# dvnam1605/MAACO-path-planing

Hardware: AMD Instinct MI355X
Metric: agent-fitness-evals/sec on 512x512 grid (higher is better)
Workload: dtype f64

## Files before the change

include/pathfit.h:

```cpp
#ifndef PATHFIT_H
#define PATHFIT_H
#include <stdint.h>
#ifdef __cplusplus
extern "C" {
#endif

#define PF_ST_OK 0
#define PF_ST_INFEASIBLE 1
#define PF_ST_STEP_CAP 2
#define PF_ST_OVERFLOW 3
#define PF_ST_KEPT 4

#define PF_ASTAR_REF 0
#define PF_ASTAR_MPA 1
#define PF_ASTAR_DIJKSTRA 2

typedef struct pf_handle pf_handle;

typedef struct {
  int32_t variant;
  int32_t restrict_policy;
  double w_turn, w_safe, min_safe, diag_pen;
} pf_score_params;

// ... 102 lines not shown
int pf_mpa_setup(pf_handle* h, const pf_mpa_params* p, const pf_score_params* sp);
int pf_mpa_phase_batch(pf_handle* h, int32_t phase, double CF, int32_t iter, uint64_t seed, int32_t n,
                       int32_t path_cap, const int32_t* d_pop_cells, const int32_t* d_pop_len,
                       const double* d_pop_stats, const int32_t* d_gidx, const int32_t* d_slot,
                       const int32_t* d_elite_cells, int32_t elite_len, const double* d_elite_stats,
                       int32_t* d_out_cells, int32_t* d_out_len, double* d_out_stats, int32_t* d_status);
int pf_mpa_fads_batch(pf_handle* h, double CF, int32_t iter, uint64_t seed, int32_t n, int32_t path_cap,
                      const int32_t* d_gidx, const int32_t* d_slot, int32_t* d_pop_cells, int32_t* d_pop_len,
                      double* d_pop_stats, int32_t* d_status);
int pf_mpa_iter_batch(pf_handle* h, int32_t phase, double CF, int32_t iter, uint64_t seed, int32_t n, int32_t path_cap,
                      int32_t* d_pop_cells, int32_t* d_pop_len, double* d_pop_stats, const int32_t* d_gidx,
                      const int32_t* d_slot, const int32_t* d_elite_cells, int32_t elite_len, const double* d_elite_stats,
                      int32_t* d_c1_cells, int32_t* d_c1_len, double* d_c1_stats, int32_t* d_c2_cells, int32_t* d_c2_len,
                      double* d_c2_stats, int32_t* d_status);
int pf_mpa_iter_ahead(pf_handle* h, int32_t depth, const int32_t* phases, const double* CFs, const int32_t* iters, uint64_t seed, int32_t n,
                      int32_t path_cap, int32_t* d_pop_cells, int32_t* d_pop_len, double* d_pop_stats, const int32_t* d_gidx,
                      const int32_t* d_slot, const int32_t* d_elite_cells, int32_t elite_len, const double* d_elite_stats,
                      int32_t* d_c1_cells, int32_t* d_c1_len, double* d_c1_stats, int32_t* d_c2_cells, int32_t* d_c2_len,
                      double* d_c2_stats, int32_t* d_status, int32_t* accepted);
int pf_mpa_ahead_take(pf_handle* h, int32_t iter, const int32_t* d_slot, int32_t* d_pop_cells, int32_t* d_pop_len, double* d_pop_stats,
                      int32_t* accepted);
int pf_mpa_ahead_level_bufs(pf_handle* h, void** out7);
int pf_mpa_ahead_drop(pf_handle* h);
int pf_mpa_ahead_stats(pf_handle* h, int64_t* out6);
int pf_mpa_rebuild_batch(pf_handle* h, int32_t iter, uint64_t seed, int32_t n, int32_t path_cap,
                         const int32_t* d_pop_cells, const int32_t* d_pop_len, const double* d_pop_stats,
                         const int32_t* d_elite_cells, int32_t elite_len, const int32_t* d_idx,
                         const int32_t* d_is_levy, const double* d_scale, const int32_t* d_agent,
                         int32_t* d_out_cells, int32_t* d_out_len, double* d_out_stats, int32_t* d_status);
int pf_mpa_memory(pf_handle* h, int32_t n, int32_t path_cap, const int32_t* d_slot, const int32_t* d_cand_cells,
                  const int32_t* d_cand_len, const double* d_cand_stats, int32_t* d_pop_cells, int32_t* d_pop_len,
                  double* d_pop_stats);

typedef struct pf_mpa_batch pf_mpa_batch;
int pf_mpa_batch_create(pf_handle* h, const pf_mpa_params* p, const pf_score_params* sp, int32_t K, const int32_t* starts,
                        const int32_t* targets, const uint64_t* seeds, pf_mpa_batch** out);
void pf_mpa_batch_destroy(pf_mpa_batch* b);
int pf_mpa_batch_init_path(pf_mpa_batch* b, int32_t k, int32_t* cells_out, int32_t cap, int32_t* len_out, double* stats5);
int pf_mpa_batch_create_ms(pf_mpa_batch* b, double* out3);
int pf_mpa_batch_sort(pf_mpa_batch* b, const double* d_pop_stats, int32_t* d_order);
int pf_mpa_batch_pick_elite(pf_mpa_batch* b, int32_t path_cap, const int32_t* d_pop_cells, const int32_t* d_pop_len,
                            const double* d_pop_stats, const int32_t* d_order);
int pf_mpa_batch_iterate(pf_mpa_batch* b, int32_t phase, double CF, int32_t iter, int32_t path_cap, int32_t* d_pop_cells,
                         int32_t* d_pop_len, double* d_pop_stats, const int32_t* d_order, int32_t* d_c1_cells, int32_t* d_c1_len,
                         double* d_c1_stats, int32_t* d_c2_cells, int32_t* d_c2_len, double* d_c2_stats, int32_t* d_status);
int pf_mpa_batch_best_rows(pf_mpa_batch* b, const double* d_pop_stats, const int32_t* d_order, double* out);
int pf_mpa_batch_read_path(pf_mpa_batch* b, int32_t k, int32_t slot, int32_t path_cap, const int32_t* d_pop_cells,
// ... 87 lines not shown
```

maaco-path-planing_amd/csrc/pathfit.hip:

```cpp
#include <hip/hip_runtime.h>
#include <dlfcn.h>
#include <rccl/rccl.h>
#include <math.h>
#include <stdio.h>
#include <stdlib.h>
#include <string.h>
#include <algorithm>
#include <chrono>
#include <queue>
#include <string>
#include <vector>

#include "../../include/pathfit.h"
#include "pf_astar.h"
#include "pf_device.h"
#include "pf_score.h"

using namespace pf;

#define DOM_MAACO 1
#define DOM_MPA 2
#define DOM_PSO 3
#define DOM_MPA_FADS 5
#define DOM_GA 4
// ... 1005 lines not shown
  Open O = make_open(smem, p.c.S, p.c.tier2);
  Slot s = slot_load(p.c, p.c.G.R * p.c.G.C);
  AStat tot = {0, 0, 0, 0, 0, 0};
  unsigned long long cells = 0, ovf = 0;
  for (;;) {
    const int a = next_agent(p.c, p.n, lane);
    if (a < 0) break;
    mpa_fads_item(p, a, s, O, tot, cells, ovf, lane);
  }
  slot_store(p.c, s, lane);
  flush_counters(p.c.cnt, tot, cells, ovf, lane);
}

struct MpaSweepArgs { MpaPhaseArgs ph; MpaFadsArgs fd; };
struct __attribute__((aligned(16))) MpaJob {
  const int* src;
  int n0;
  int astart, g0, g1;
  int kind;
  int aux;
};
struct MpaRes { int n, rc; };

PF_DEV void mpa_plan_item(const MpaPhaseArgs& p, const MpaFadsArgs& f, bool isph, int a, int item, MpaJob* jobs, MpaRes* res) {
  const Grid& G = p.c.G;
  const int lane = lane_id();
  MpaJob j; j.src = nullptr; j.n0 = 0; j.astart = 0; j.g0 = -1; j.g1 = p.m.target; j.kind = 0; j.aux = isph ? 4 : 0;
  unsigned long long pruned_n = 0;
  if (isph) {
    const MpaPlan pl = mpa_plan(p, a);
    const int2 pr = p.prop[a];
    const int idx = first_i(pr.x);
    if (idx >= 0) {
      const int* mod = pl.mod;
      const int cur = mod[idx];
      const int inter = first_i(pr.y);
      bool pruned = false;
      if (p.m.dt) {
        double pre = 0.0;
        for (int i = lane; i < idx; i += 64) {
          const int dd = mod[i + 1] - mod[i];
          pre += (dd == 1 || dd == -1 || dd == G.C || dd == -G.C) ? 1.0 : PF_SQRT2;
        }
        pre = wave_sum_d(pre);
        double lb = p.m.dt[cur];
        if (G.occ[inter] != 1 && inter != cur) {
          const int r0 = row_of(G, cur), r1 = row_of(G, inter);
          const long dr_ = r1 - r0, dc_ = (inter - r1 * G.C) - (cur - r0 * G.C);
          lb = fmin(lb, __builtin_sqrt((double)(dr_ * dr_ + dc_ * dc_)) + p.m.dt[inter]);
        }
        lb = (pre + lb) * (1.0 - 1e-9);
        const double prey_fit = pl.prey_stats[4];
        pruned = lb >= prey_fit && (mod == pl.prey || pl.mod_stats[4] >= prey_fit);
      }
      if (pruned) pruned_n = 1;
      else if (idx + 1 > p.path_cap) j.aux = 3;
      else {
        j.kind = 1; j.src = mod; j.n0 = idx + 1; j.astart = cur;
        j.g0 = (G.occ[inter] != 1 && inter != cur) ? inter : -1;
      }
    }
  } else {
    Rng g; g.init(f.seed, DOM_MPA_FADS, (unsigned long long)f.iter, (unsigned long long)f.gidx[a]);
    if (g.random() < f.m.fads) {
      if (g.random() < f.CF) {
        const int rr_ = (int)g.randint(0, G.R - 1);
        const int rc_ = (int)g.randint(0, G.C - 1);
        const int node = rr_ * G.C + rc_;
        bool pruned = false;
        if (f.m.dt && G.occ[node] != 1) {
          pruned = (f.m.ds[node] + f.m.dt[node]) * (1.0 - 1e-9) >= f.pop_stats[(size_t)f.slot[a] * 5 + 4];
          if (pruned) pruned_n = 1;
        }
        if (G.occ[node] != 1 && !pruned) { j.kind = 2; j.n0 = 0; j.astart = f.m.start; j.g0 = node; }
      } else if (f.init_len > 0) j.aux = f.init_len > f.path_cap ? 3 : 1;
    }
  }
  if (lane == 0) {
    jobs[item] = j;
    MpaRes r; r.n = 0; r.rc = 1; res[item] = r;
    if (pruned_n) atomicAdd(&p.c.cnt->pruned, pruned_n);
  }
}
__global__ __launch_bounds__(64) void k_mpa_plan(MpaSweepArgs q, MpaJob* jobs, MpaRes* res) {
  const MpaPhaseArgs& p = q.ph;
  const int item = blockIdx.x;
  if (item >= 2 * p.n) return;
  const bool isph = item < p.n;
  mpa_plan_item(p, q.fd, isph, isph ? item : item - p.n, item, jobs, res);
}

struct MpaSearchArgs { Common c; const MpaJob* jobs; MpaRes* res; int n_items, path_cap; int* ph_cells; int* fd_cells; int n; };

template <bool PR>
__global__ __launch_bounds__(PR ? 128 : 64) __attribute__((amdgpu_waves_per_eu(3, 8))) void k_mpa_search(MpaSearchArgs p) {
  extern __shared__ __attribute__((aligned(16))) char smem[];
  const int lane = lane_id();
  const Grid& G = p.c.G;
  const int RC = G.R * G.C;
#ifdef PF_TWO_WAVE
  if (PR) {
    const int wave = (int)(threadIdx.x >> 6);
    if (wave == 0) pr_init_ctl(smem, lane);
    __syncthreads();
// ... 2740 lines not shown
  CK(hipMemsetAsync(h->d_scan3, 0, sizeof(int), h->stream));
  hipLaunchKernelGGL(k_plan_decode_multi<>, dim3((a.n + 255) / 256), dim3(256), 0, h->stream, a.c.G, a.n, a.W, a.wp_cells, a.wp_pos, d_start, d_target,
                     est, (int*)h->d_scan3);
  CK(hipGetLastError());
  return 0;
}
static int decode_multi_bad_ends(pf_handle* h, int* bad) {
  if (d2h_one(h, (const int*)h->d_scan3, bad)) return -1;
  h->d2h_small += 1;
  return 0;
}
static int decode_multi_launch(pf_handle* h, const DecodeArgs& a, const int* d_start, const int* d_target, int n) {
  DecodeMultiArgs m;
  m.c = a.c; m.sp = a.sp; m.do_score = a.do_score; m.n = a.n; m.W = a.W; m.path_cap = a.path_cap; m.start = d_start; m.target = d_target;
  m.wp_cells = a.wp_cells; m.wp_pos = a.wp_pos; m.cells = a.cells; m.len = a.len; m.status = a.status; m.stats = a.stats;
  return plateau_map(h) ? launch_with_retry(h, k_decode_multi<true>, m, n) : launch_with_retry(h, k_decode_multi<false>, m, n);
}

#include "pf_mpa_ahead.h"

struct MpaAhead {
  int *c1_cells = nullptr, *c1_len = nullptr, *c2_cells = nullptr, *c2_len = nullptr, *status = nullptr;
  double *c1_stats = nullptr, *c2_stats = nullptr;
  size_t rows_cap = 0; int row_cells = 0;
  unsigned long long* d_ctl = nullptr;
  int planned = 0, valid = 0, next = 0;
  int prev_accepted = 0;
  int iters[PF_AHEAD_MAX] = {};
  int n = 0, path_cap = 0;
  const int* slot = nullptr; int* pop_cells = nullptr; int* pop_len = nullptr; double* pop_stats = nullptr;
  int last_level = -1;
  long long sweeps = 0, levels = 0, served = 0, stale = 0;
};
static void mpa_ahead_drop(pf_handle* h) {
  MpaAhead* S = h->ahead;
  if (!S) return;
  S->planned = S->valid = S->next = 0; S->last_level = -1;
}
static void mpa_ahead_free(pf_handle* h) {
  MpaAhead* S = h->ahead;
  if (!S) return;
  void* ptrs[] = {S->c1_cells, S->c1_len, S->c1_stats, S->c2_cells, S->c2_len, S->c2_stats, S->status, S->d_ctl};
  for (void* q : ptrs) if (q) (void)hipFree(q);
  delete S;
  h->ahead = nullptr;
}
static int mpa_ahead_state(pf_handle* h) {
  if (!h->ahead) h->ahead = new MpaAhead();
  if (!h->ahead->d_ctl) CK(hipMalloc(&h->ahead->d_ctl, sizeof(unsigned long long) * (1 + PF_AHEAD_MAX)));
  return 0;
}
static int mpa_ahead_rows(pf_handle* h, size_t rows, int path_cap) {
  MpaAhead* S = h->ahead;
  if (rows <= S->rows_cap && path_cap == S->row_cells) return 0;
  CK(hipStreamSynchronize(h->stream));
  void** slots[] = {(void**)&S->c1_cells, (void**)&S->c1_len, (void**)&S->c1_stats, (void**)&S->c2_cells, (void**)&S->c2_len,
                    (void**)&S->c2_stats, (void**)&S->status};
  for (void** q : slots) if (*q) { (void)hipFree(*q); *q = nullptr; }
  S->rows_cap = 0;
  CK(hipMalloc(&S->c1_cells, sizeof(int) * rows * path_cap)); CK(hipMalloc(&S->c2_cells, sizeof(int) * rows * path_cap));
  CK(hipMalloc(&S->c1_len, sizeof(int) * rows)); CK(hipMalloc(&S->c2_len, sizeof(int) * rows)); CK(hipMalloc(&S->status, sizeof(int) * rows));
  CK(hipMalloc(&S->c1_stats, sizeof(double) * 5 * rows)); CK(hipMalloc(&S->c2_stats, sizeof(double) * 5 * rows));
  S->rows_cap = rows; S->row_cells = path_cap;
  return 0;
}

extern "C" {

int pf_mpa_iter_ahead(pf_handle* h, int32_t depth, const int32_t* phases, const double* CFs, const int32_t* iters, uint64_t seed, int32_t n,
                      int32_t path_cap, int32_t* d_pop_cells, int32_t* d_pop_len, double* d_pop_stats, const int32_t* d_gidx,
                      const int32_t* d_slot, const int32_t* d_elite_cells, int32_t elite_len, const double* d_elite_stats,
                      int32_t* d_c1_cells, int32_t* d_c1_len, double* d_c1_stats, int32_t* d_c2_cells, int32_t* d_c2_len,
                      double* d_c2_stats, int32_t* d_status, int32_t* accepted) {
  if (!h) return -2;
  if (!h->mpa_ready) return failmsg(h, "pf_mpa_iter_ahead: call pf_mpa_setup first");
  if (depth < 1 || depth > PF_AHEAD_MAX || !phases || !CFs || !iters || n <= 0 || (int64_t)depth * n > (1 << 28) || path_cap < 2 || !d_pop_cells ||
      !d_pop_len || !d_pop_stats || !d_gidx || !d_slot || !d_elite_cells || !d_elite_stats || !d_c1_cells || !d_c1_len || !d_c1_stats ||
      !d_c2_cells || !d_c2_len || !d_c2_stats || !d_status || !accepted)
    return failmsg(h, "pf_mpa_iter_ahead: bad arguments");
  for (int d = 0; d < depth; ++d) if (phases[d] < 1 || phases[d] > 3) return failmsg(h, "pf_mpa_iter_ahead: bad arguments");
  MpaBase base;
  if (mpa_solo_base(h, &base) || mpa_ahead_state(h)) return -1;
  mpa_ahead_drop(h);
  MpaAhead* S = h->ahead;
  const int D = depth, DN = D * n;
  if (D > 1) {
    if (mpa_ahead_rows(h, (size_t)DN, path_cap)) return -1;
    d_c1_cells = S->c1_cells; d_c1_len = S->c1_len; d_c1_stats = S->c1_stats;
    d_c2_cells = S->c2_cells; d_c2_len = S->c2_len; d_c2_stats = S->c2_stats; d_status = S->status;
  }
  MpaLevels ls; ls.D = D; ls.N = n;
  for (int d = 0; d < PF_AHEAD_MAX; ++d) { const int e = d < D ? d : 0; ls.lv[d].phase = phases[e]; ls.lv[d].iter = iters[e]; ls.lv[d].CF = CFs[e]; }
  MpaSweepArgs a;
  a.ph = mpa_phase_args(base, phases[0], CFs[0], iters[0], seed, n, path_cap, d_pop_cells, d_pop_len, d_pop_stats, d_gidx, d_slot, d_c1_cells,
                        d_c1_len, d_c1_stats, d_status);
  a.ph.elite_cells = d_elite_cells; a.ph.elite_len = elite_len; a.ph.elite_stats = d_elite_stats;
  if (elite_len < 0) { if (ensure_elite_buf(h)) return -1; a.ph.elite_len_dev = h->d_elite_len; }
  a.fd = mpa_fads_args(base, CFs[0], iters[0], seed, n, path_cap, d_pop_cells, d_pop_len, d_pop_stats, d_gidx, d_slot, d_status);
  a.fd.init_cells = h->d_init_cells; a.fd.init_len = h->init_len; a.fd.init_stats = h->d_init_stats;
  a.fd.cand_cells = d_c2_cells; a.fd.cand_len = d_c2_len; a.fd.cand_stats = d_c2_stats;
  int prc = 0;
  if (make_queue(h, 2 * DN, [&](float* est) {
        if (D == 1) {
          prc = mpa_launch_propose(h, a.ph, est);
          hipLaunchKernelGGL(k_plan_mpa_fads, dim3((n + 255) / 256), dim3(256), 0, h->stream, a.fd, est + n);
          return;
        }
        prc = mpa_prop_scratch(h, a.ph, DN);
        if (prc) return;
        hipLaunchKernelGGL(k_mpa_estimates_ahead<>, dim3((2 * DN + 255) / 256), dim3(256), 0, h->stream, a.ph, a.fd, ls, est);
      })) return -1;
  if (prc) return -1;
  {
    std::vector<int> list;
    if (mpa_doubt_list(h, a.ph, list)) return -1;
    for (int g : list) {
      const int d = g / n;
      MpaPhaseArgs v = a.ph;
      level_view(v, ls, d);
      if (mpa_resolve_one(h, v, g - d * n)) return -1;
    }
  }
#ifdef PF_TWO_WAVE
  const bool pr = g_two_wave != 0 && !plateau_map(h);
#else
  const bool pr = false;
#endif
  unsigned long long* const ctl = S->d_ctl;
  if (D > 1) CK(hipMemsetAsync(ctl, 0, sizeof(unsigned long long) * (1 + PF_AHEAD_MAX), h->stream));
  DevCounters dc;
  if (mpa_launch_sweep(h, a, DN, pr,
      [&](MpaJob* jobs, MpaRes* jres) {
        if (D == 1) hipLaunchKernelGGL(k_mpa_plan, dim3(2 * n), dim3(64), 0, h->stream, a, jobs, jres);
        else hipLaunchKernelGGL(k_mpa_plan_ahead<>, dim3(2 * DN), dim3(64), 0, h->stream, a, ls, jobs, jres);
      },
      [&](const MpaJob* jobs, const MpaRes* jres) {
        if (D == 1) hipLaunchKernelGGL(k_mpa_finish, dim3(2 * n), dim3(64), 0, h->stream, a, jobs, jres);
        else hipLaunchKernelGGL(k_mpa_finish_ahead<>, dim3(2 * DN), dim3(64), 0, h->stream, a, ls, jobs, jres, ctl + 1);
      },
      [&] { hipLaunchKernelGGL(k_mpa_apply_count<>, dim3(n), dim3(64), 0, h->stream, n, path_cap, d_slot, (const int*)d_c1_cells, (const int*)d_c1_len,
                               (const double*)d_c1_stats, (const int*)d_c2_cells, (const int*)d_c2_len, (const double*)d_c2_stats, d_pop_cells,
                               d_pop_len, d_pop_stats, &h->d_cnt->done); },
      &dc)) return -1;
  *accepted = (int32_t)dc.done;
  if (D == 1) return 0;
  unsigned long long hc[1 + PF_AHEAD_MAX];
  if (d2h_bytes(h, ctl, hc, sizeof(unsigned long long) * (size_t)(1 + D))) return -1;
  h->d2h_small += 1;
  h->last.overflow_agents = (long long)hc[1];
  S->sweeps += 1; S->levels += D - 1;
  S->planned = D; S->valid = D; S->next = 1; S->prev_accepted = (int)dc.done; S->last_level = 0;
  for (int d = D - 1; d >= 1; --d) if (hc[1 + d] > 0) S->valid = d;
  if (hc[1] > 0) S->valid = 1;
  for (int d = 0; d < D; ++d) S->iters[d] = iters[d];
  S->n = n; S->path_cap = path_cap; S->slot = d_slot; S->pop_cells = d_pop_cells; S->pop_len = d_pop_len; S->pop_stats = d_pop_stats;
  return 0;
}

int pf_mpa_ahead_take(pf_handle* h, int32_t iter, const int32_t* d_slot, int32_t* d_pop_cells, int32_t* d_pop_len, double* d_pop_stats,
                      int32_t* accepted) {
  if (!h) return -2;
  if (!accepted) return failmsg(h, "pf_mpa_ahead_take: bad arguments");
  *accepted = -1;
  MpaAhead* S = h->ahead;
  if (!S || S->next >= S->planned) return 0;
  const int d = S->next;
  if (d >= S->valid || S->prev_accepted != 0 || S->iters[d] != iter || d_slot != S->slot || d_pop_cells != S->pop_cells ||
      d_pop_len != S->pop_len || d_pop_stats != S->pop_stats) {
    S->stale += 1;
    mpa_ahead_drop(h);
    return 0;
  }
  CK(hipSetDevice(h->device));
  const size_t o = (size_t)d * (size_t)S->n;
  const int n = S->n, cap = S->path_cap;
  CK(hipMemsetAsync(S->d_ctl, 0, sizeof(unsigned long long), h->stream));
  hipLaunchKernelGGL(k_mpa_apply_count<>, dim3(n), dim3(64), 0, h->stream, n, cap, d_slot, (const int*)(S->c1_cells + o * cap),
                     (const int*)(S->c1_len + o), (const double*)(S->c1_stats + o * 5), (const int*)(S->c2_cells + o * cap), (const int*)(S->c2_len + o),
                     (const double*)(S->c2_stats + o * 5), d_pop_cells, d_pop_len, d_pop_stats, S->d_ctl);
  CK(hipGetLastError());
  unsigned long long acc64 = 0;
  if (d2h_one(h, S->d_ctl, &acc64)) return -1;
  h->d2h_small += 1;
  const int acc = (int)acc64;
  S->prev_accepted = acc; S->next = d + 1; S->last_level = d; S->served += 1;
  h->last = pf_counters{}; h->last_ms = 0.f;
  *accepted = acc;
  return 0;
}

int pf_mpa_ahead_level_bufs(pf_handle* h, void** out7) {
  if (!h) return -2;
  if (!out7) return failmsg(h, "pf_mpa_ahead_level_bufs: bad arguments");
  for (int i = 0; i < 7; ++i) out7[i] = nullptr;
  const MpaAhead* S = h->ahead;
  if (!S || S->last_level < 0) return 0;
  const size_t o = (size_t)S->last_level * (size_t)S->n;
  out7[0] = S->c1_cells + o * S->path_cap; out7[1] = S->c1_len + o; out7[2] = S->c1_stats + o * 5;
  out7[3] = S->c2_cells + o * S->path_cap; out7[4] = S->c2_len + o; out7[5] = S->c2_stats + o * 5; out7[6] = S->status + o;
  return 0;
}

int pf_mpa_ahead_drop(pf_handle* h) { if (!h) return -2; mpa_ahead_drop(h); return 0; }

int pf_mpa_ahead_stats(pf_handle* h, int64_t* out6) {
  if (!h) return -2;
  if (!out6) return failmsg(h, "pf_mpa_ahead_stats: bad arguments");
  const MpaAhead* S = h->ahead;
  out6[0] = g_mpa_lookahead; out6[1] = g_mpa_lookahead_always;
  out6[2] = S ? S->sweeps : 0; out6[3] = S ? S->levels : 0; out6[4] = S ? S->served : 0; out6[5] = S ? S->stale : 0;
  return 0;
}

}

#include "pf_pso_batch.h"
extern "C" {

int pf_pso_update_batch(pf_handle* h, int32_t n, int32_t K, int32_t N, int32_t W, double w, double c1, double c2, double max_vel, uint64_t iter,
                        const uint64_t* d_seeds, const int32_t* d_tab, const int32_t* d_starts, const int32_t* d_targets, const double* d_pos,
                        const double* d_vel, const double* d_pbest, const double* d_gbest, double* d_s_pos, double* d_s_vel, int32_t* d_s_start,
                        int32_t* d_s_target, int32_t* d_s_row) {
  if (!h) return -2;
  if (n < 0 || K < 1 || N < 1 || (int64_t)K * N > (1 << 29) || n > K * N || W < 1 || (int64_t)n * W > (1ll << 31) - 256 || !d_seeds || !d_tab || !d_starts ||
      !d_targets || !d_pos || !d_vel || !d_pbest || !d_gbest || !d_s_pos || !d_s_vel || !d_s_start || !d_s_target || !d_s_row)
    return failmsg(h, "pf_pso_update_batch: bad arguments (0 <= n <= K * N <= 2^29)");
  if (n == 0) return 0;
  CK(hipSetDevice(h->device));
  PsoArgs a{n, W, h->R, h->C, w, c1, c2, max_vel, const_cast<double*>(d_pos), const_cast<double*>(d_vel), d_pbest, d_gbest, 0ull, iter, 0ull, nullptr, nullptr};
  const int threads = 256, blocks = (n * W + threads - 1) / threads;
  hipLaunchKernelGGL(k_pso_update_batch<>, dim3(blocks), dim3(threads), 0, h->stream, a, K, N, (const unsigned long long*)d_seeds, d_tab, d_starts, d_targets,
                     d_s_pos, d_s_vel, d_s_start, d_s_target, d_s_row);
  CK(hipGetLastError());
// ... 41 lines not shown
```

maaco-path-planing_amd/csrc/pf_mpa_ahead.h:

```cpp
#define PF_AHEAD_MAX 16
struct MpaLevel { int phase, iter; double CF; };
struct MpaLevels { MpaLevel lv[PF_AHEAD_MAX]; int D, N; };

__host__ __device__ __forceinline__ void level_view(MpaPhaseArgs& p, const MpaLevels& ls, int d) {
  const size_t o = (size_t)d * (size_t)ls.N;
  p.phase = ls.lv[d].phase; p.iter = ls.lv[d].iter; p.CF = ls.lv[d].CF;
  p.out_cells += o * p.path_cap; p.out_len += o; p.out_stats += o * 5; p.status += o;
  p.prop += o;
}
__host__ __device__ __forceinline__ void level_view(MpaFadsArgs& f, const MpaLevels& ls, int d) {
  const size_t o = (size_t)d * (size_t)ls.N;
  f.iter = ls.lv[d].iter; f.CF = ls.lv[d].CF;
  f.status += o;
  f.cand_cells += o * f.path_cap; f.cand_len += o; f.cand_stats += o * 5;
}

template <int PF_LATE = 0>
__global__ void k_mpa_estimates_ahead(MpaPhaseArgs p0, MpaFadsArgs f0, MpaLevels ls, float* est) {
  const int DN = ls.D * ls.N;
  const int t = blockIdx.x * blockDim.x + threadIdx.x;
  if (t >= 2 * DN) return;
  const bool isph = t < DN;
  const int g = isph ? t : t - DN;
  const int d = g / ls.N, a = g - d * ls.N;
  if (isph) {
    MpaPhaseArgs p = p0;
    level_view(p, ls, d);
    mpa_propose_item(p, a, g, est + (size_t)d * ls.N);
  } else {
    MpaFadsArgs f = f0;
    level_view(f, ls, d);
    mpa_fads_est_item(f, a, est + (size_t)DN + (size_t)d * ls.N);
  }
}
template <int PF_LATE = 0>
__global__ __launch_bounds__(64) void k_mpa_plan_ahead(MpaSweepArgs q, MpaLevels ls, MpaJob* jobs, MpaRes* res) {
  const int DN = ls.D * ls.N;
  const int item = blockIdx.x;
  if (item >= 2 * DN) return;
  const bool isph = item < DN;
  const int g = isph ? item : item - DN;
  const int d = g / ls.N, a = g - d * ls.N;
  MpaPhaseArgs p = q.ph; MpaFadsArgs f = q.fd;
  level_view(p, ls, d); level_view(f, ls, d);
  mpa_plan_item(p, f, isph, a, item, jobs, res);
}
template <int PF_LATE = 0>
__global__ __launch_bounds__(64) void k_mpa_finish_ahead(MpaSweepArgs q, MpaLevels ls, const MpaJob* jobs, const MpaRes* res,
                                                         unsigned long long* lvl_ovf) {
  const int DN = ls.D * ls.N;
  const int item = blockIdx.x;
  if (item >= 2 * DN) return;
  const bool isph = item < DN;
  const int g = isph ? item : item - DN;
  const int d = g / ls.N, a = g - d * ls.N;
  MpaPhaseArgs p = q.ph; MpaFadsArgs f = q.fd;
  level_view(p, ls, d); level_view(f, ls, d);
  mpa_finish_item(p, f, isph, a, item, jobs, res);
  if (threadIdx.x == 0) {
    const MpaJob j = jobs[item];
    if (j.kind != 0 ? res[item].rc == 3 : j.aux == 3) atomicAdd(&lvl_ovf[d], 1ull);
  }
}
template <int PF_LATE = 0>
__global__ __launch_bounds__(64) void k_mpa_apply_count(int n, int path_cap, const int* slots, const int* c1_cells, const int* c1_len,
                                                        const double* c1_stats, const int* c2_cells, const int* c2_len,
                                                        const double* c2_stats, int* pop_cells, int* pop_len, double* pop_stats,
                                                        unsigned long long* accepted) {
  const int a = blockIdx.x;
  if (a >= n) return;
  const int slot = slots[a];
  const double fit = pop_stats[(size_t)slot * 5 + 4];
  const bool take = c1_stats[(size_t)a * 5 + 4] < fit || (c2_len[a] > 0 && c2_stats[(size_t)a * 5 + 4] < fit);
  __syncthreads();
  if (!take) return;
  if (threadIdx.x == 0) atomicAdd(accepted, 1ull);
  mpa_apply_item(a, slot, path_cap, c1_cells, c1_len, c1_stats, c2_cells, c2_len, c2_stats, pop_cells, pop_len, pop_stats);
}
```

maaco-path-planing_amd/pathfit/engine.py:

```python
import ctypes as C

import numpy as np

from . import _lib
from ._lib import Counters, MaacoParams, MpaParams, PathfitError, ScoreParams

INF = float("inf")
ST_OK, ST_INFEASIBLE, ST_STEP_CAP, ST_OVERFLOW, ST_KEPT = 0, 1, 2, 3, 4


class DevBuf:

    def __init__(self, eng, shape, dtype):
        self.eng = eng
        self.shape = tuple(int(s) for s in (shape if isinstance(shape, (tuple, list)) else (shape,)))
        self.dtype = np.dtype(dtype)
        self.nbytes = int(np.prod(self.shape, dtype=np.int64)) * self.dtype.itemsize
        p = C.c_void_p()
        eng._ck(eng.L.pf_dev_alloc(eng.h, self.nbytes, C.byref(p)))
        self.ptr = p.value

    def upload(self, arr):
        a = np.ascontiguousarray(arr, self.dtype)
        assert a.nbytes <= self.nbytes, (a.nbytes, self.nbytes)
# ... 373 lines not shown

    def mpa_ahead_take(self, it, d_slot, d_pop_cells, d_pop_len, d_pop_stats):
        acc = C.c_int32(-1)
        self._ck(self.L.pf_mpa_ahead_take(self.h, int(it), d_slot.ptr, d_pop_cells.ptr, d_pop_len.ptr, d_pop_stats.ptr, C.byref(acc)))
        return acc.value

    def mpa_ahead_level_bufs(self, n, path_cap):
        out = (C.c_void_p * 7)()
        self._ck(self.L.pf_mpa_ahead_level_bufs(self.h, C.addressof(out)))
        if not out[0]:
            return None
        shapes = [((n, path_cap), np.int32), ((n,), np.int32), ((n, 5), np.float64)] * 2 + [((n,), np.int32)]
        views = []
        for p, (shape, dt) in zip(out, shapes):
            v = _View(self, p, int(np.prod(shape)), dt)
            v.shape = shape
            views.append(v)
        return views

    def mpa_ahead_drop(self):
        self._ck(self.L.pf_mpa_ahead_drop(self.h))

    def mpa_ahead_stats(self):
        out = (C.c_int64 * 6)()
        self._ck(self.L.pf_mpa_ahead_stats(self.h, C.addressof(out)))
        return dict(zip(("cap", "always", "merged_sweeps", "levels_ahead", "served", "stale"), (int(v) for v in out)))

    def ga_select(self, seed, gen, n, k, d_fit_all, d_gorder, d_psid):
        self._ck(self.L.pf_ga_select_dev(self.h, int(seed), int(gen), int(n), int(k), d_fit_all.ptr, d_gorder.ptr, d_psid.ptr))

    def ga_breed(self, seed, gen, N, W, cx, mut, d_chrom_all, d_psid, child0, nchild, d_out):
        self._ck(self.L.pf_ga_breed_dev(self.h, int(seed), int(gen), int(N), int(W), float(cx), float(mut), d_chrom_all.ptr, d_psid.ptr,
                                        int(child0), int(nchild), d_out.ptr))

    def ga_assemble(self, n_loc, W, cap, lo, kid_len, kid_chrom, kid_stats, kid_cells, psid, chrom_old, stats_old, cells_old, len_old,
                    old_lo, old_hi, chrom_new, stats_new, cells_new, len_new):
        self._ck(self.L.pf_ga_assemble_dev(self.h, int(n_loc), int(W), int(cap), int(lo), kid_len.ptr, kid_chrom.ptr, kid_stats.ptr,
                                           kid_cells.ptr, psid.ptr, chrom_old.ptr, stats_old.ptr, cells_old.ptr, len_old.ptr,
                                           int(old_lo), int(old_hi), chrom_new.ptr, stats_new.ptr, cells_new.ptr, len_new.ptr))

    def ga_select_batch(self, d_seeds, gen, K, N, k, d_fit_all, d_gorder, d_psid):
        self._ck(self.L.pf_ga_select_batch(self.h, d_seeds.ptr, int(gen), int(K), int(N), int(k), d_fit_all.ptr, d_gorder.ptr, d_psid.ptr))

    def ga_breed_batch(self, d_seeds, gen, K, N, W, cx, mut, d_chrom_all, d_psid, d_out):
        self._ck(self.L.pf_ga_breed_batch(self.h, d_seeds.ptr, int(gen), int(K), int(N), int(W), float(cx), float(mut), d_chrom_all.ptr,
                                          d_psid.ptr, d_out.ptr))

    def ga_assemble_batch(self, K, N, W, cap, kid_len, kid_chrom, kid_stats, kid_cells, psid, chrom_old, stats_old, cells_old, len_old,
                          chrom_new, stats_new, cells_new, len_new):
# ... 63 lines not shown
```

maaco-path-planing_amd/pathfit/mpa.py:

```python
import math

import numpy as np

from ._lib import MpaParams
from .engine import Engine, score_params
from .env import START_NODE_VAL, TARGET_NODE_VAL, find_marker
from .paths import CellPath

INF = float("inf")


def levy_sigma(beta):
    num = math.gamma(1 + beta) * math.sin(math.pi * beta / 2)
    den = math.gamma((1 + beta) / 2) * beta * (2 ** ((beta - 1) / 2))
    return (num / den) ** (1 / beta) if den > 1e-9 else 1.0


def cf_and_phase(it, num_iterations):
    ratio = it / num_iterations
    CF = 0.0 if ratio >= 1.0 else ((1.0 - ratio) ** (2.0 * ratio) if ratio > 0 else 1.0)
    phase = 1 if it <= num_iterations / 3 else (2 if it <= 2 * num_iterations / 3 else 3)
    return CF, phase


STALE = -1


def lookahead_depth(history, cap, left, always=False):
    if cap <= 0:
        return 0
    if left <= 1:
        return 1
    if history and history[-1] == STALE:
        return 1
    quiet = always or (len(history) > 0 and history[-1] == 0)
    return min(int(cap), int(left)) if quiet else 1


class BestSoFar:

    def _init_best(self):
        self.best_path_overall = []
        self.best_path_length_overall = INF
        self.best_path_turns_overall = INF
        self.best_safety_penalty_overall = INF
        self.best_diag_penalty_overall = INF
        self.best_fitness_overall = INF
        self.convergence_curve_data = []

    def _update_best(self, s, fetch):
        self.best_fitness_overall = float(s[4])
        self.best_path_overall = fetch()
        self.best_path_length_overall = float(s[0])
        self.best_path_turns_overall = int(s[1])
        self.best_safety_penalty_overall = float(s[2])
        self.best_diag_penalty_overall = float(s[3])

    def _take_first(self, s, fetch):
        self._update_best(s, fetch)
# ... 146 lines not shown
        return s

    def drop_lookahead(self):
        self.accept_history = []
        self._ahead_left = 0
        if hasattr(self.engine, "mpa_ahead_drop"):
            self.engine.mpa_ahead_drop()

    def _sweep(self, it, n, d_gidx, d_slot, world=1):
        e, cap, K = self.engine, self.path_cap, self.num_iterations
        own = self._own_rows
        st = e.mpa_ahead_stats() if world == 1 else {"cap": 0, "always": 0}
        el_c, el_s = self._el_cells.ptr, self._el_stats.ptr
        CF, phase = cf_and_phase(it, K)
        acc, rows = -1, own
        if st["cap"] > 0 and self._ahead_left > 0:
            acc = e.mpa_ahead_take(it, d_slot, self.d_cells, self.d_len, self.d_stats)
            self._ahead_left = self._ahead_left - 1 if acc >= 0 else 0
            if acc < 0:
                self.accept_history.append(STALE)
            else:
                rows = None
        if acc < 0:
            depth = lookahead_depth(self.accept_history, st["cap"], K - it + 1, bool(st["always"]))
            if depth == 0:
                self._ahead_left = 0
                e.mpa_iter(phase, CF, it, self.seed, n, cap, self.d_cells, self.d_len, self.d_stats, d_gidx, d_slot, el_c, -1, el_s, *own)
            else:
                levels = [(cf_and_phase(it + d, K)[1], cf_and_phase(it + d, K)[0], it + d) for d in range(depth)]
                acc = e.mpa_iter_ahead(levels, self.seed, n, cap, self.d_cells, self.d_len, self.d_stats, d_gidx, d_slot, el_c, -1,
                                       el_s, *own)
                self._ahead_left = depth - 1
                if depth > 1:
                    rows = None
        if acc >= 0:
            self.accept_history.append(acc)
        (self.d_cand_cells, self.d_cand_len, self.d_cand_stats, self.d_c2_cells, self.d_c2_len, self.d_c2_stats,
         self.d_status) = rows or e.mpa_ahead_level_bufs(n, cap)

    def _check_overflow(self):
        n = self.engine.counters()["overflow_agents"]
        if n:
            raise RuntimeError("pathfit: scratch/path capacity overflow on %d predators (path_cap=%d)" % (n, self.path_cap))

    def solve_path_planning(self):
        self._sort()
        slot, s0 = self._best_row()
# ... 7 lines not shown
```

Before: 348,500.

## Speculate MPA phase-3 lookahead levels with elite snapshot validation and late pruning

Extends the multi-iteration lookahead so that phase-3 levels can be computed speculatively even when the previous iteration accepted changes. At plan time the kernel stores pruning bounds instead of pruning, and it snapshots the elite row. When a speculative level is consumed, new kernels check that the elite is unchanged and apply the bound-based pruning late against the current population. This is meant to cut per-iteration sweeps and host round trips in phase 3. The cost is wasted speculative work whenever the elite changes, plus extra kernels and buffers.

```diff
diff --git a/include/pathfit.h b/include/pathfit.h
--- a/include/pathfit.h
+++ b/include/pathfit.h
@@ -148,7 +148,7 @@
                       int32_t* accepted);
 int pf_mpa_ahead_level_bufs(pf_handle* h, void** out7);
 int pf_mpa_ahead_drop(pf_handle* h);
-int pf_mpa_ahead_stats(pf_handle* h, int64_t* out6);
+int pf_mpa_ahead_stats(pf_handle* h, int64_t* out8);
 int pf_mpa_rebuild_batch(pf_handle* h, int32_t iter, uint64_t seed, int32_t n, int32_t path_cap,
                          const int32_t* d_pop_cells, const int32_t* d_pop_len, const double* d_pop_stats,
                          const int32_t* d_elite_cells, int32_t elite_len, const int32_t* d_idx,
diff --git a/maaco-path-planing_amd/csrc/pathfit.hip b/maaco-path-planing_amd/csrc/pathfit.hip
--- a/maaco-path-planing_amd/csrc/pathfit.hip
+++ b/maaco-path-planing_amd/csrc/pathfit.hip
@@ -1051,11 +1051,35 @@
 };
 struct MpaRes { int n, rc; };
 
-PF_DEV void mpa_plan_item(const MpaPhaseArgs& p, const MpaFadsArgs& f, bool isph, int a, int item, MpaJob* jobs, MpaRes* res) {
+PF_DEV double mpa_phase_bound(const Grid& G, const MpaDev& m, const int* mod, int idx, int cur, int inter, int lane) {
+  double pre = 0.0;
+  for (int i = lane; i < idx; i += 64) {
+    const int dd = mod[i + 1] - mod[i];
+    pre += (dd == 1 || dd == -1 || dd == G.C || dd == -G.C) ? 1.0 : PF_SQRT2;
+  }
+  pre = wave_sum_d(pre);
+  double lb = m.dt[cur];
+  if (G.occ[inter] != 1 && inter != cur) {
+    const int r0 = row_of(G, cur), r1 = row_of(G, inter);
+    const long dr_ = r1 - r0, dc_ = (inter - r1 * G.C) - (cur - r0 * G.C);
+    lb = fmin(lb, __builtin_sqrt((double)(dr_ * dr_ + dc_ * dc_)) + m.dt[inter]);
+  }
+  return (pre + lb) * (1.0 - 1e-9);
+}
+PF_DEV bool mpa_phase_prunes(double lb, double prey_fit, bool mod_is_prey, double mod_fit) {
+  return lb >= prey_fit && (mod_is_prey || mod_fit >= prey_fit);
+}
+PF_DEV double mpa_fads_bound(const MpaDev& m, int node) { return (m.ds[node] + m.dt[node]) * (1.0 - 1e-9); }
+PF_DEV bool mpa_fads_prunes(double lb, double fit) { return lb >= fit; }
+#define PF_NO_BOUND (-PF_INF)
+
+PF_DEV void mpa_plan_item(const MpaPhaseArgs& p, const MpaFadsArgs& f, bool isph, int a, int item, MpaJob* jobs, MpaRes* res,
+                          double* keep_bound = nullptr) {
   const Grid& G = p.c.G;
   const int lane = lane_id();
   MpaJob j; j.src = nullptr; j.n0 = 0; j.astart = 0; j.g0 = -1; j.g1 = p.m.target; j.kind = 0; j.aux = isph ? 4 : 0;
   unsigned long long pruned_n = 0;
+  double bound = PF_NO_BOUND;
   if (isph) {
     const MpaPlan pl = mpa_plan(p, a);
     const int2 pr = p.prop[a];
@@ -1066,21 +1090,8 @@
       const int inter = first_i(pr.y);
       bool pruned = false;
       if (p.m.dt) {
-        double pre = 0.0;
-        for (int i = lane; i < idx; i += 64) {
-          const int dd = mod[i + 1] - mod[i];
-          pre += (dd == 1 || dd == -1 || dd == G.C || dd == -G.C) ? 1.0 : PF_SQRT2;
-        }
-        pre = wave_sum_d(pre);
-        double lb = p.m.dt[cur];
-        if (G.occ[inter] != 1 && inter != cur) {
-          const int r0 = row_of(G, cur), r1 = row_of(G, inter);
-          const long dr_ = r1 - r0, dc_ = (inter - r1 * G.C) - (cur - r0 * G.C);
-          lb = fmin(lb, __builtin_sqrt((double)(dr_ * dr_ + dc_ * dc_)) + p.m.dt[inter]);
-        }
-        lb = (pre + lb) * (1.0 - 1e-9);
-        const double prey_fit = pl.prey_stats[4];
-        pruned = lb >= prey_fit && (mod == pl.prey || pl.mod_stats[4] >= prey_fit);
+        bound = mpa_phase_bound(G, p.m, mod, idx, cur, inter, lane);
+        pruned = !keep_bound && mpa_phase_prunes(bound, pl.prey_stats[4], mod == pl.prey, pl.mod_stats[4]);
       }
       if (pruned) pruned_n = 1;
       else if (idx + 1 > p.path_cap) j.aux = 3;
@@ -1098,7 +1109,8 @@
         const int node = rr_ * G.C + rc_;
         bool pruned = false;
         if (f.m.dt && G.occ[node] != 1) {
-          pruned = (f.m.ds[node] + f.m.dt[node]) * (1.0 - 1e-9) >= f.pop_stats[(size_t)f.slot[a] * 5 + 4];
+          bound = mpa_fads_bound(f.m, node);
+          pruned = !keep_bound && mpa_fads_prunes(bound, f.pop_stats[(size_t)f.slot[a] * 5 + 4]);
           if (pruned) pruned_n = 1;
         }
         if (G.occ[node] != 1 && !pruned) { j.kind = 2; j.n0 = 0; j.astart = f.m.start; j.g0 = node; }
@@ -1109,6 +1121,7 @@
     jobs[item] = j;
     MpaRes r; r.n = 0; r.rc = 1; res[item] = r;
     if (pruned_n) atomicAdd(&p.c.cnt->pruned, pruned_n);
+    if (keep_bound) *keep_bound = bound;
   }
 }
 __global__ __launch_bounds__(64) void k_mpa_plan(MpaSweepArgs q, MpaJob* jobs, MpaRes* res) {
@@ -3895,15 +3908,19 @@
 struct MpaAhead {
   int *c1_cells = nullptr, *c1_len = nullptr, *c2_cells = nullptr, *c2_len = nullptr, *status = nullptr;
   double *c1_stats = nullptr, *c2_stats = nullptr;
+  double* bound = nullptr;
+  int *snap_cells = nullptr, *snap_len = nullptr; double* snap_stats = nullptr;
   size_t rows_cap = 0; int row_cells = 0;
   unsigned long long* d_ctl = nullptr;
   int planned = 0, valid = 0, next = 0;
-  int prev_accepted = 0;
+  bool quiet = true;
+  unsigned spec = 0;
+  MpaEliteRow elite = {};
   int iters[PF_AHEAD_MAX] = {};
   int n = 0, path_cap = 0;
   const int* slot = nullptr; int* pop_cells = nullptr; int* pop_len = nullptr; double* pop_stats = nullptr;
   int last_level = -1;
-  long long sweeps = 0, levels = 0, served = 0, stale = 0;
+  long long sweeps = 0, levels = 0, served = 0, stale = 0, served_elite = 0, stale_elite = 0;
 };
 static void mpa_ahead_drop(pf_handle* h) {
   MpaAhead* S = h->ahead;
@@ -3913,7 +3930,8 @@
 static void mpa_ahead_free(pf_handle* h) {
   MpaAhead* S = h->ahead;
   if (!S) return;
-  void* ptrs[] = {S->c1_cells, S->c1_len, S->c1_stats, S->c2_cells, S->c2_len, S->c2_stats, S->status, S->d_ctl};
+  void* ptrs[] = {S->c1_cells, S->c1_len, S->c1_stats, S->c2_cells, S->c2_len, S->c2_stats, S->status, S->d_ctl, S->bound, S->snap_cells,
+                  S->snap_len, S->snap_stats};
   for (void* q : ptrs) if (q) (void)hipFree(q);
   delete S;
   h->ahead = nullptr;
@@ -3921,6 +3939,7 @@
 static int mpa_ahead_state(pf_handle* h) {
   if (!h->ahead) h->ahead = new MpaAhead();
   if (!h->ahead->d_ctl) CK(hipMalloc(&h->ahead->d_ctl, sizeof(unsigned long long) * (1 + PF_AHEAD_MAX)));
+  if (!h->ahead->snap_len) { CK(hipMalloc(&h->ahead->snap_len, sizeof(int))); CK(hipMalloc(&h->ahead->snap_stats, sizeof(double) * 5)); }
   return 0;
 }
 static int mpa_ahead_rows(pf_handle* h, size_t rows, int path_cap) {
@@ -3928,12 +3947,13 @@
   if (rows <= S->rows_cap && path_cap == S->row_cells) return 0;
   CK(hipStreamSynchronize(h->stream));
   void** slots[] = {(void**)&S->c1_cells, (void**)&S->c1_len, (void**)&S->c1_stats, (void**)&S->c2_cells, (void**)&S->c2_len,
-                    (void**)&S->c2_stats, (void**)&S->status};
+                    (void**)&S->c2_stats, (void**)&S->status, (void**)&S->bound, (void**)&S->snap_cells};
   for (void** q : slots) if (*q) { (void)hipFree(*q); *q = nullptr; }
   S->rows_cap = 0;
   CK(hipMalloc(&S->c1_cells, sizeof(int) * rows * path_cap)); CK(hipMalloc(&S->c2_cells, sizeof(int) * rows * path_cap));
   CK(hipMalloc(&S->c1_len, sizeof(int) * rows)); CK(hipMalloc(&S->c2_len, sizeof(int) * rows)); CK(hipMalloc(&S->status, sizeof(int) * rows));
   CK(hipMalloc(&S->c1_stats, sizeof(double) * 5 * rows)); CK(hipMalloc(&S->c2_stats, sizeof(double) * 5 * rows));
+  CK(hipMalloc(&S->bound, sizeof(double) * 2 * rows)); CK(hipMalloc(&S->snap_cells, sizeof(int) * (size_t)path_cap));
   S->rows_cap = rows; S->row_cells = path_cap;
   return 0;
 }
@@ -3962,7 +3982,8 @@
     d_c1_cells = S->c1_cells; d_c1_len = S->c1_len; d_c1_stats = S->c1_stats;
     d_c2_cells = S->c2_cells; d_c2_len = S->c2_len; d_c2_stats = S->c2_stats; d_status = S->status;
   }
-  MpaLevels ls; ls.D = D; ls.N = n;
+  MpaLevels ls; ls.D = D; ls.N = n; ls.spec = 0;
+  if (elite_len < 0) for (int d = 1; d < D; ++d) if (phases[d] == 3) ls.spec |= 1u << d;
   for (int d = 0; d < PF_AHEAD_MAX; ++d) { const int e = d < D ? d : 0; ls.lv[d].phase = phases[e]; ls.lv[d].iter = iters[e]; ls.lv[d].CF = CFs[e]; }
   MpaSweepArgs a;
   a.ph = mpa_phase_args(base, phases[0], CFs[0], iters[0], seed, n, path_cap, d_pop_cells, d_pop_len, d_pop_stats, d_gidx, d_slot, d_c1_cells,
@@ -4001,11 +4022,16 @@
 #endif
   unsigned long long* const ctl = S->d_ctl;
   if (D > 1) CK(hipMemsetAsync(ctl, 0, sizeof(unsigned long long) * (1 + PF_AHEAD_MAX), h->stream));
+  const MpaEliteRow elite = {d_elite_cells, a.ph.elite_len_dev, d_elite_stats};
+  if (ls.spec) {
+    hipLaunchKernelGGL(k_mpa_elite_snap<>, dim3(1), dim3(256), 0, h->stream, elite, path_cap, S->snap_cells, S->snap_len, S->snap_stats);
+    CK(hipGetLastError());
+  }
   DevCounters dc;
   if (mpa_launch_sweep(h, a, DN, pr,
       [&](MpaJob* jobs, MpaRes* jres) {
         if (D == 1) hipLaunchKernelGGL(k_mpa_plan, dim3(2 * n), dim3(64), 0, h->stream, a, jobs, jres);
-        else hipLaunchKernelGGL(k_mpa_plan_ahead<>, dim3(2 * DN), dim3(64), 0, h->stream, a, ls, jobs, jres);
+        else hipLaunchKernelGGL(k_mpa_plan_ahead<>, dim3(2 * DN), dim3(64), 0, h->stream, a, ls, jobs, jres, S->bound);
       },
       [&](const MpaJob* jobs, const MpaRes* jres) {
         if (D == 1) hipLaunchKernelGGL(k_mpa_finish, dim3(2 * n), dim3(64), 0, h->stream, a, jobs, jres);
@@ -4013,7 +4039,7 @@
       },
       [&] { hipLaunchKernelGGL(k_mpa_apply_count<>, dim3(n), dim3(64), 0, h->stream, n, path_cap, d_slot, (const int*)d_c1_cells, (const int*)d_c1_len,
                                (const double*)d_c1_stats, (const int*)d_c2_cells, (const int*)d_c2_len, (const double*)d_c2_stats, d_pop_cells,
-                               d_pop_len, d_pop_stats, &h->d_cnt->done); },
+                               d_pop_len, d_pop_stats, &h->d_cnt->done, (const unsigned long long*)nullptr); },
       &dc)) return -1;
   *accepted = (int32_t)dc.done;
   if (D == 1) return 0;
@@ -4022,7 +4048,7 @@
   h->d2h_small += 1;
   h->last.overflow_agents = (long long)hc[1];
   S->sweeps += 1; S->levels += D - 1;
-  S->planned = D; S->valid = D; S->next = 1; S->prev_accepted = (int)dc.done; S->last_level = 0;
+  S->planned = D; S->valid = D; S->next = 1; S->quiet = dc.done == 0; S->last_level = 0; S->spec = ls.spec; S->elite = elite;
   for (int d = D - 1; d >= 1; --d) if (hc[1 + d] > 0) S->valid = d;
   if (hc[1] > 0) S->valid = 1;
   for (int d = 0; d < D; ++d) S->iters[d] = iters[d];
@@ -4038,26 +4064,42 @@
   MpaAhead* S = h->ahead;
   if (!S || S->next >= S->planned) return 0;
   const int d = S->next;
-  if (d >= S->valid || S->prev_accepted != 0 || S->iters[d] != iter || d_slot != S->slot || d_pop_cells != S->pop_cells ||
+  const bool spec = (S->spec >> d) & 1u;
+  if (d >= S->valid || (!spec && !S->quiet) || S->iters[d] != iter || d_slot != S->slot || d_pop_cells != S->pop_cells ||
       d_pop_len != S->pop_len || d_pop_stats != S->pop_stats) {
-    S->stale += 1;
+    S->stale += 1; S->stale_elite += spec;
     mpa_ahead_drop(h);
     return 0;
   }
   CK(hipSetDevice(h->device));
   const size_t o = (size_t)d * (size_t)S->n;
   const int n = S->n, cap = S->path_cap;
-  CK(hipMemsetAsync(S->d_ctl, 0, sizeof(unsigned long long), h->stream));
-  hipLaunchKernelGGL(k_mpa_apply_count<>, dim3(n), dim3(64), 0, h->stream, n, cap, d_slot, (const int*)(S->c1_cells + o * cap),
-                     (const int*)(S->c1_len + o), (const double*)(S->c1_stats + o * 5), (const int*)(S->c2_cells + o * cap), (const int*)(S->c2_len + o),
-                     (const double*)(S->c2_stats + o * 5), d_pop_cells, d_pop_len, d_pop_stats, S->d_ctl);
+  unsigned long long* const ctl = S->d_ctl;
+  int* const c1_cells = S->c1_cells + o * cap; int* const c1_len = S->c1_len + o; double* const c1_stats = S->c1_stats + o * 5;
+  int* const c2_len = S->c2_len + o;
+  if (spec) {
+    hipLaunchKernelGGL(k_mpa_elite_same<>, dim3(1), dim3(256), 0, h->stream, S->elite, cap, (const int*)S->snap_cells, (const int*)S->snap_len,
+                       (const double*)S->snap_stats, ctl);
+    const size_t DN = (size_t)S->planned * (size_t)n;
+    hipLaunchKernelGGL(k_mpa_prune_late<>, dim3(2 * n), dim3(64), 0, h->stream, n, cap, d_slot, (const double*)d_pop_stats, S->elite,
+                       (const double*)(S->bound + o), (const double*)(S->bound + DN + o), c1_cells, c1_len, c1_stats, S->status + o, c2_len, ctl);
+  } else CK(hipMemsetAsync(ctl, 0, sizeof(unsigned long long), h->stream));
+  hipLaunchKernelGGL(k_mpa_apply_count<>, dim3(n), dim3(64), 0, h->stream, n, cap, d_slot, (const int*)c1_cells, (const int*)c1_len,
+                     (const double*)c1_stats, (const int*)(S->c2_cells + o * cap), (const int*)c2_len, (const double*)(S->c2_stats + o * 5),
+                     d_pop_cells, d_pop_len, d_pop_stats, ctl, (const unsigned long long*)ctl);
   CK(hipGetLastError());
-  unsigned long long acc64 = 0;
-  if (d2h_one(h, S->d_ctl, &acc64)) return -1;
+  unsigned long long word = 0;
+  if (d2h_one(h, ctl, &word)) return -1;
   h->d2h_small += 1;
-  const int acc = (int)acc64;
-  S->prev_accepted = acc; S->next = d + 1; S->last_level = d; S->served += 1;
+  if (word & PF_CTL_STALE) {
+    S->stale += 1; S->stale_elite += 1;
+    mpa_ahead_drop(h);
+    return 0;
+  }
+  const int acc = (int)(word & ((1ull << PF_CTL_PRUNED_SHIFT) - 1));
+  S->quiet = S->quiet && acc == 0; S->next = d + 1; S->last_level = d; S->served += 1; S->served_elite += spec;
   h->last = pf_counters{}; h->last_ms = 0.f;
+  h->last.pruned_rebuilds = (long long)((word & ~PF_CTL_STALE) >> PF_CTL_PRUNED_SHIFT);
   *accepted = acc;
   return 0;
 }
@@ -4076,12 +4118,13 @@
 
 int pf_mpa_ahead_drop(pf_handle* h) { if (!h) return -2; mpa_ahead_drop(h); return 0; }
 
-int pf_mpa_ahead_stats(pf_handle* h, int64_t* out6) {
-  if (!h) return -2;
-  if (!out6) return failmsg(h, "pf_mpa_ahead_stats: bad arguments");
+int pf_mpa_ahead_stats(pf_handle* h, int64_t* out8) {
+  if (!h) return -2;
+  if (!out8) return failmsg(h, "pf_mpa_ahead_stats: bad arguments");
   const MpaAhead* S = h->ahead;
-  out6[0] = g_mpa_lookahead; out6[1] = g_mpa_lookahead_always;
-  out6[2] = S ? S->sweeps : 0; out6[3] = S ? S->levels : 0; out6[4] = S ? S->served : 0; out6[5] = S ? S->stale : 0;
+  out8[0] = g_mpa_lookahead; out8[1] = g_mpa_lookahead_always;
+  out8[2] = S ? S->sweeps : 0; out8[3] = S ? S->levels : 0; out8[4] = S ? S->served : 0; out8[5] = S ? S->stale : 0;
+  out8[6] = S ? S->served_elite : 0; out8[7] = S ? S->stale_elite : 0;
   return 0;
 }
 
diff --git a/maaco-path-planing_amd/csrc/pf_mpa_ahead.h b/maaco-path-planing_amd/csrc/pf_mpa_ahead.h
--- a/maaco-path-planing_amd/csrc/pf_mpa_ahead.h
+++ b/maaco-path-planing_amd/csrc/pf_mpa_ahead.h
@@ -1,6 +1,6 @@
 #define PF_AHEAD_MAX 16
 struct MpaLevel { int phase, iter; double CF; };
-struct MpaLevels { MpaLevel lv[PF_AHEAD_MAX]; int D, N; };
+struct MpaLevels { MpaLevel lv[PF_AHEAD_MAX]; int D, N; unsigned spec; };
 
 __host__ __device__ __forceinline__ void level_view(MpaPhaseArgs& p, const MpaLevels& ls, int d) {
   const size_t o = (size_t)d * (size_t)ls.N;
@@ -34,7 +34,7 @@
   }
 }
 template <int PF_LATE = 0>
-__global__ __launch_bounds__(64) void k_mpa_plan_ahead(MpaSweepArgs q, MpaLevels ls, MpaJob* jobs, MpaRes* res) {
+__global__ __launch_bounds__(64) void k_mpa_plan_ahead(MpaSweepArgs q, MpaLevels ls, MpaJob* jobs, MpaRes* res, double* bound) {
   const int DN = ls.D * ls.N;
   const int item = blockIdx.x;
   if (item >= 2 * DN) return;
@@ -43,7 +43,7 @@
   const int d = g / ls.N, a = g - d * ls.N;
   MpaPhaseArgs p = q.ph; MpaFadsArgs f = q.fd;
   level_view(p, ls, d); level_view(f, ls, d);
-  mpa_plan_item(p, f, isph, a, item, jobs, res);
+  mpa_plan_item(p, f, isph, a, item, jobs, res, (ls.spec >> d) & 1u ? bound + item : nullptr);
 }
 template <int PF_LATE = 0>
 __global__ __launch_bounds__(64) void k_mpa_finish_ahead(MpaSweepArgs q, MpaLevels ls, const MpaJob* jobs, const MpaRes* res,
@@ -62,13 +62,16 @@
     if (j.kind != 0 ? res[item].rc == 3 : j.aux == 3) atomicAdd(&lvl_ovf[d], 1ull);
   }
 }
+#define PF_CTL_STALE (1ull << 63)
+#define PF_CTL_PRUNED_SHIFT 31
 template <int PF_LATE = 0>
 __global__ __launch_bounds__(64) void k_mpa_apply_count(int n, int path_cap, const int* slots, const int* c1_cells, const int* c1_len,
                                                         const double* c1_stats, const int* c2_cells, const int* c2_len,
                                                         const double* c2_stats, int* pop_cells, int* pop_len, double* pop_stats,
-                                                        unsigned long long* accepted) {
+                                                        unsigned long long* accepted, const unsigned long long* gate) {
   const int a = blockIdx.x;
   if (a >= n) return;
+  if (gate && (*gate & PF_CTL_STALE)) return;
   const int slot = slots[a];
   const double fit = pop_stats[(size_t)slot * 5 + 4];
   const bool take = c1_stats[(size_t)a * 5 + 4] < fit || (c2_len[a] > 0 && c2_stats[(size_t)a * 5 + 4] < fit);
@@ -77,3 +80,44 @@
   if (threadIdx.x == 0) atomicAdd(accepted, 1ull);
   mpa_apply_item(a, slot, path_cap, c1_cells, c1_len, c1_stats, c2_cells, c2_len, c2_stats, pop_cells, pop_len, pop_stats);
 }
+
+struct MpaEliteRow { const int* cells; const int* len; const double* stats; };
+template <int PF_LATE = 0>
+__global__ __launch_bounds__(256) void k_mpa_elite_snap(MpaEliteRow e, int path_cap, int* snap_cells, int* snap_len, double* snap_stats) {
+  const int L = *e.len;
+  for (int i = threadIdx.x; i < L && i < path_cap; i += blockDim.x) snap_cells[i] = e.cells[i];
+  if (threadIdx.x < 5) snap_stats[threadIdx.x] = e.stats[threadIdx.x];
+  if (threadIdx.x == 0) *snap_len = L;
+}
+template <int PF_LATE = 0>
+__global__ __launch_bounds__(256) void k_mpa_elite_same(MpaEliteRow e, int path_cap, const int* snap_cells, const int* snap_len,
+                                                        const double* snap_stats, unsigned long long* ctl) {
+  const int L = *e.len;
+  int diff = L != *snap_len;
+  if (!diff) for (int i = threadIdx.x; i < L && i < path_cap; i += blockDim.x) diff |= snap_cells[i] != e.cells[i];
+  if (threadIdx.x < 5) diff |= __double_as_longlong(snap_stats[threadIdx.x]) != __double_as_longlong(e.stats[threadIdx.x]);
+  diff = __syncthreads_or(diff);
+  if (threadIdx.x == 0) *ctl = diff ? PF_CTL_STALE : 0ull;
+}
+template <int PF_LATE = 0>
+__global__ __launch_bounds__(64) void k_mpa_prune_late(int n, int path_cap, const int* slots, const double* pop_stats, MpaEliteRow e,
+                                                       const double* bound_ph, const double* bound_fd, int* c1_cells, int* c1_len,
+                                                       double* c1_stats, int* status, int* c2_len, unsigned long long* ctl) {
+  const int item = blockIdx.x;
+  if (item >= 2 * n || (*ctl & PF_CTL_STALE)) return;
+  const int lane = threadIdx.x;
+  const bool isph = item < n;
+  const int a = isph ? item : item - n;
+  const double fit = pop_stats[(size_t)slots[a] * 5 + 4];
+  if (isph) {
+    if (!mpa_phase_prunes(bound_ph[a], fit, false, e.stats[4])) return;
+    const int L = *e.len;
+    copy_path(c1_cells + (size_t)a * path_cap, e.cells, L < path_cap ? L : path_cap, lane);
+    if (lane < 5) c1_stats[(size_t)a * 5 + lane] = e.stats[lane];
+    if (lane == 0) { c1_len[a] = L; status[a] = 4; }
+  } else {
+    if (!mpa_fads_prunes(bound_fd[a], fit)) return;
+    if (lane == 0) c2_len[a] = 0;
+  }
+  if (lane == 0) atomicAdd(ctl, 1ull << PF_CTL_PRUNED_SHIFT);
+}
diff --git a/maaco-path-planing_amd/pathfit/engine.py b/maaco-path-planing_amd/pathfit/engine.py
--- a/maaco-path-planing_amd/pathfit/engine.py
+++ b/maaco-path-planing_amd/pathfit/engine.py
@@ -419,9 +419,10 @@
         self._ck(self.L.pf_mpa_ahead_drop(self.h))
 
     def mpa_ahead_stats(self):
-        out = (C.c_int64 * 6)()
+        out = (C.c_int64 * 8)()
         self._ck(self.L.pf_mpa_ahead_stats(self.h, C.addressof(out)))
-        return dict(zip(("cap", "always", "merged_sweeps", "levels_ahead", "served", "stale"), (int(v) for v in out)))
+        return dict(zip(("cap", "always", "merged_sweeps", "levels_ahead", "served", "stale", "served_elite", "stale_elite"),
+                        (int(v) for v in out)))
 
     def ga_select(self, seed, gen, n, k, d_fit_all, d_gorder, d_psid):
         self._ck(self.L.pf_ga_select_dev(self.h, int(seed), int(gen), int(n), int(k), d_fit_all.ptr, d_gorder.ptr, d_psid.ptr))
diff --git a/maaco-path-planing_amd/pathfit/mpa.py b/maaco-path-planing_amd/pathfit/mpa.py
--- a/maaco-path-planing_amd/pathfit/mpa.py
+++ b/maaco-path-planing_amd/pathfit/mpa.py
@@ -26,15 +26,22 @@
 STALE = -1
 
 
-def lookahead_depth(history, cap, left, always=False):
+def lookahead_depth(history, cap, left, always=False, phase3_next=0):
     if cap <= 0:
         return 0
     if left <= 1:
         return 1
+    elite = min(int(cap), int(left), 1 + max(0, int(phase3_next)))
     if history and history[-1] == STALE:
-        return 1
+        return elite
     quiet = always or (len(history) > 0 and history[-1] == 0)
-    return min(int(cap), int(left)) if quiet else 1
+    return min(int(cap), int(left)) if quiet else elite
+
+
+def phase3_after(it, num_iterations):
+    if it >= num_iterations or cf_and_phase(it + 1, num_iterations)[1] != 3:
+        return 0
+    return num_iterations - it
 
 
 class BestSoFar:
@@ -227,7 +234,7 @@
             else:
                 rows = None
         if acc < 0:
-            depth = lookahead_depth(self.accept_history, st["cap"], K - it + 1, bool(st["always"]))
+            depth = lookahead_depth(self.accept_history, st["cap"], K - it + 1, bool(st["always"]), phase3_after(it, K))
             if depth == 0:
                 self._ahead_left = 0
                 e.mpa_iter(phase, CF, it, self.seed, n, cap, self.d_cells, self.d_len, self.d_stats, d_gidx, d_slot, el_c, -1, el_s, *own)
```

After: 336,800. -3.3%, worse.
